# garrelt/C2-Ray3Dm

Hardware: AMD Instinct MI355X
Metric: cells-traced/sec (grid^3 x sources / wallclock) on 256^3 (higher is better)
Workload: dtype f64

## Files before the change

c2-ray3dm_amd/csrc/kernels_common.hpp:

```cpp
#pragma once
#include <hip/hip_runtime.h>
#include <stdint.h>

namespace c2r {

#ifndef C2R_BLOCK
#define C2R_BLOCK 256
#endif
constexpr int kFusedQmaxK = 10;
constexpr int kBlock = C2R_BLOCK;

typedef double v2f64 __attribute__((ext_vector_type(2)));
constexpr int kLogTab = 64;

struct ShellStep { double d2axis[3]; double path_scale, lls_scale; };
struct ChemStep { double dt, brech0, acolh0, recpow, clumping, sqrtt, expt, zp, dzdt; };
struct StepBlock {
    double dr[3], dr2[3], vol, coldensh_LLS, inv_dr0;
    int exact_udiv_dr0, n_shell;
    ChemStep chem;
};

struct KParams {
    int n[3];
// ... 5 lines not shown
    double inv_dlogtau;
    int exact_udiv;
    int numtau;
    int R, P;
    size_t PP;
    const double *nhi, *nhi_T;
    double *phih;
    double *phih_T;
    int lls_type;
    double R_max2;
    const float *lls, *lls_T;
    double *gbox_h;
    double *gbox;
    const double *thick, *thin;
    const double *hthick, *hthin;
    double *heat, *heat_T;
    double tau_heat_limit;
    const v2f64 *logtab;
    const v2f64 *odtab;
    double od_per_e, od_per_ln;
    const int    *srcpos;
    const int    *srcw;
    const double *normflux;
    const double *xthick, *xthin;
    const double *xhthick, *xhthin;
    const double *normflux_x;
    double *planes;
};

struct FaceRect {
    int a_lo, wa, b_lo, wb;
    unsigned magic;
    int ntiles;
    int pp, npr;
};

struct ShellArgs {
    int q;
    int has_boundary;
    int buf_prev, buf_cur;
    int tiles_max;
    int boxR[3], boxL[3];
    double alam;
    double dp2, inv_dp2;
    double inv_q;
    FaceRect face[6];
    const int *active;
    const int *n_active;
    double *loss_partial;
    double *dbg_cdout;
};

__device__ __forceinline__ int pmod(int a, int n) { int r = a % n; return r < 0 ? r + n : r; }

#define C2R_AS4 __attribute__((address_space(4)))
__device__ __forceinline__ const C2R_AS4 StepBlock &step_of(const KParams &p) { return *(const C2R_AS4 StepBlock *)p.step; }
__device__ __forceinline__ const C2R_AS4 ShellStep &shell_step(const KParams &p, int q) { return ((const C2R_AS4 ShellStep *)p.shell_step)[q]; }

__device__ __forceinline__ double rcp_nr(double d)
{
    double r = __builtin_amdgcn_rcp(d);
    double e = __builtin_fma(-d, r, 1.0);
    r = __builtin_fma(r, e, r);
    e = __builtin_fma(-d, r, 1.0);
    return __builtin_fma(r, e, r);
}
__device__ __forceinline__ double fdiv(double n, double d)
{
    const double r = rcp_nr(d);
    const double q = n * r;
    const double rem = __builtin_fma(-d, q, n);
    return __builtin_fma(rem, r, q);
}
__device__ __forceinline__ double frcp(double d)
{
    const double r = rcp_nr(d);
    const double rem = __builtin_fma(-d, r, 1.0);
    return __builtin_fma(rem, r, r);
}
__device__ __forceinline__ double fsqrt(double x)
{
#ifdef C2R_SQRT_GENERIC
    return sqrt(x);
#else
    const double y = __builtin_amdgcn_rsq(x);
    double g = x * y;
    double h = y * 0.5;
    const double r = __builtin_fma(-h, g, 0.5);
    g = __builtin_fma(g, r, g);
    h = __builtin_fma(h, r, h);
    double d = __builtin_fma(-g, g, x);
    g = __builtin_fma(d, h, g);
    d = __builtin_fma(-g, g, x);
    return __builtin_fma(d, h, g);
#endif
}
__device__ __forceinline__ double udiv(double n, double d, double rd, int exact)
{
    if (!exact) return n / d;
    const double q = n * rd;
    const double r = __builtin_fma(-q, d, n);
    return __builtin_fma(r, rd, q);
}

__device__ __forceinline__ double log10_pos(double x)
{
#ifdef C2R_LOG10_OCML
    return log10(x);
#else
    double m = __builtin_amdgcn_frexp_mant(x);
    int e = __builtin_amdgcn_frexp_exp(x);
    const bool lo = m < 0.70710678118654752440;
    m = lo ? m + m : m;
    e = lo ? e - 1 : e;
    const double dk = (double)e;
    const double f = m - 1.0;
    const double s = f * rcp_nr(2.0 + f);
    const double z = s * s, w = z * z;
    const double t1 = w * __builtin_fma(w, __builtin_fma(w, 1.531383769920937332e-01, 2.222219843214978396e-01),
                                        3.999999999940941908e-01);
    const double t2 = z * __builtin_fma(w, __builtin_fma(w, __builtin_fma(w, 1.479819860511658591e-01,
                                        1.818357216161805012e-01), 2.857142874366239149e-01),
                                        6.666666666666735130e-01);
    const double R = t2 + t1;
    const double hfsq = 0.5 * f * f;
    const double lm = f - (hfsq - s * (hfsq + R));
    const double hi = __builtin_fma(lm, 4.34294481903251816668e-01, dk * 3.01029995663611771306e-01);
    return __builtin_fma(dk, 3.69423907715893078616e-13, hi);
#endif
}

__device__ __forceinline__ double log10_tab(double x, const v2f64 *__restrict__ tab)
{
    const double m = __builtin_amdgcn_frexp_mant(x);
    const int e = __builtin_amdgcn_frexp_exp(x);
    const unsigned i = ((unsigned)__double2hiint(m) >> 14) & 63u;
    const v2f64 rt = tab[i];
    const double z = __builtin_fma(m, rt.x, -1.0);
    double P = __builtin_fma(z, 1.0 / 7.0, -1.0 / 6.0);
    P = __builtin_fma(z, P, 0.2);
    P = __builtin_fma(z, P, -0.25);
    P = __builtin_fma(z, P, 1.0 / 3.0);
    P = __builtin_fma(z, P, -0.5);
    const double l1p = __builtin_fma(z * z, P, z);
    return __builtin_fma((double)e, 3.01029995663981198017e-01, __builtin_fma(l1p, 4.34294481903251816668e-01, rt.y));
}
__device__ __forceinline__ const v2f64 *wave_log_table(const v2f64 *__restrict__ g, v2f64 *lds )
{
    const unsigned tid = threadIdx.x, lane = tid & 63u;
    v2f64 *mine = lds + (tid & ~63u);
    mine[lane] = g[lane];
    return mine;
}

struct TauPos { int ip, ip1; double res; };
__device__ __forceinline__ TauPos tau_pos(double tau, const KParams &p, const v2f64 *__restrict__ ltab)
{
#ifdef C2R_LOG10_NOTAB
    const double lt = log10_pos(fmax(1.0e-20, tau));
#else
    const double lt = log10_tab(fmax(1.0e-20, tau), ltab);
#endif
    const double od = fmin(p.numtau_d, fmax(0.0, 1.0 + udiv(lt - p.minlogtau, p.dlogtau, p.inv_dlogtau, p.exact_udiv)));
    TauPos t;
    t.ip = (int)od;
    t.res = od - (double)t.ip;
    t.ip1 = min(p.numtau, t.ip + 1);
    return t;
}
__device__ __forceinline__ double read_table(const double *__restrict__ tab, const TauPos &t)
{
    typedef double d2u __attribute__((ext_vector_type(2), aligned(8)));
    const d2u v = *reinterpret_cast<const d2u *>(tab + t.ip);
    return v.x + (v.y - v.x) * t.res;
}

template <int EXT = 0>
__device__ __forceinline__ double photoion(const KParams &p, const v2f64 *__restrict__ ltab, double cd_in, double cd_out,
                                           double vol_ph, double nflux, double &p_out, double *heat = nullptr, double nflux_x = 0.0)
{
    const double tau_in = cd_in * p.sigma, tau_out = cd_out * p.sigma;
    const TauPos pin = tau_pos(tau_in, p, ltab);
    const double p_in = nflux * read_table(p.thick, pin);
    double p_cell;
    TauPos pout = pin;
    const bool thick_cell = fabs(tau_out - tau_in) > p.tau_limit;
    if (thick_cell) {
        pout = tau_pos(tau_out, p, ltab);
        p_out = nflux * read_table(p.thick, pout);
        p_cell = p_in - p_out;
    } else {
        p_cell = nflux * (tau_out - tau_in) * read_table(p.thin, pin);
        p_out = p_in - p_cell;
    }
    if (EXT & 1) {
        const double h_in = nflux * read_table(p.hthick, pin);
        if (fabs(tau_out - tau_in) > p.tau_heat_limit) {
            if (!thick_cell) pout = tau_pos(tau_out, p, ltab);
            *heat = fdiv(h_in - nflux * read_table(p.hthick, pout), vol_ph);
        } else {
            const double tau_cell = (cd_out - cd_in) * p.sigma;
            *heat = fdiv(nflux * tau_cell * read_table(p.hthin, pin), vol_ph);
        }
    }
    double rate = fdiv(p_cell, vol_ph);
    if ((EXT & 2) && nflux_x > 0.0) {
        const double x_in = nflux_x * read_table(p.xthick, pin);
        double x_cell, x_out;
        if (thick_cell) {
            x_out = nflux_x * read_table(p.xthick, pout);
            x_cell = x_in - x_out;
        } else {
            x_cell = nflux_x * (tau_out - tau_in) * read_table(p.xthin, pin);
            x_out = x_in - x_cell;
        }
        p_out = p_out + x_out;
        rate = rate + fdiv(x_cell, vol_ph);
        if (EXT & 1) {
            const double hx_in = nflux_x * read_table(p.xhthick, pin);
            if (fabs(tau_out - tau_in) > p.tau_heat_limit) *heat = *heat + fdiv(hx_in - nflux_x * read_table(p.xhthick, pout), vol_ph);
            else *heat = *heat + fdiv(nflux_x * ((cd_out - cd_in) * p.sigma) * read_table(p.xhthin, pin), vol_ph);
        }
    }
    return rate;
}

__device__ __forceinline__ double block_sum_256(double v, double *sm )
{
    for (int off = 32; off > 0; off >>= 1) v += __shfl_down(v, off, 64);
    const int tid = threadIdx.y * blockDim.x + threadIdx.x;
    const int wave = tid >> 6, lane = tid & 63;
    if (lane == 0) sm[wave] = v;
    __syncthreads();
    double r = 0.0;
    if (tid == 0) { const int nw = (blockDim.x * blockDim.y) >> 6; for (int w = 0; w < nw; ++w) r += sm[w]; }
    return r;
}

__device__ __forceinline__ double rcp1(double d)
{
    const double r = __builtin_amdgcn_rcp(d);
    return __builtin_fma(__builtin_fma(-d, r, 1.0), r, r);
}
__device__ __forceinline__ double tau_od(double tau, const KParams &p, const v2f64 *__restrict__ tab)
{
    const double x = fmax(1.0e-20, tau);
    const double m = __builtin_amdgcn_frexp_mant(x);
    const int e = __builtin_amdgcn_frexp_exp(x);
    const unsigned i = ((unsigned)__double2hiint(m) >> 14) & 63u;
    const v2f64 rt = tab[i];
    const double z = __builtin_fma(m, rt.x, -1.0);
    double P = __builtin_fma(z, 1.0 / 7.0, -1.0 / 6.0);
    P = __builtin_fma(z, P, 0.2);
    P = __builtin_fma(z, P, -0.25);
    P = __builtin_fma(z, P, 1.0 / 3.0);
    P = __builtin_fma(z, P, -0.5);
    const double l1p = __builtin_fma(z * z, P, z);
    const double od = __builtin_fma((double)e, p.od_per_e, __builtin_fma(l1p, p.od_per_ln, rt.y));
    return fmin(p.numtau_d, od);
}
__device__ __forceinline__ double table_at(const double *__restrict__ tab, double od)
{
    typedef double d2u __attribute__((ext_vector_type(2), aligned(8)));
    const d2u v = *reinterpret_cast<const d2u *>(tab + (int)od);
    return __builtin_fma(v.y - v.x, __builtin_amdgcn_fract(od), v.x);
}

template <int EXT>
__device__ __forceinline__ double rates_fast(const KParams &p, const v2f64 *__restrict__ ltab, const double *__restrict__ thick,
                                             const double cd_in, const double cd_out, const double nflux, const double nflux_x,
                                             const double volnhi, const double vol_ph, double &p_out, double &heat)
{
    const double tau_in = cd_in * p.sigma, tau_out = cd_out * p.sigma;
    const double od_in = tau_od(tau_in, p, ltab);
    const double t_in = table_at(thick, od_in);
    double dT, t_out, od_out = od_in;
    const bool thick_cell = fabs(tau_out - tau_in) > p.tau_limit;
    if (thick_cell) {
        od_out = tau_od(tau_out, p, ltab);
        t_out = table_at(thick, od_out);
        dT = t_in - t_out;
    } else {
        dT = (tau_out - tau_in) * table_at(p.thin, od_in);
        t_out = t_in - dT;
    }
    p_out = nflux * t_out;
    if (EXT & 1) {
        const double h_in = table_at(p.hthick, od_in);
        double dH;
        if (fabs(tau_out - tau_in) > p.tau_heat_limit) {
            if (!thick_cell) od_out = tau_od(tau_out, p, ltab);
            dH = h_in - table_at(p.hthick, od_out);
        } else dH = ((cd_out - cd_in) * p.sigma) * table_at(p.hthin, od_in);
        heat = (nflux * dH) * rcp1(vol_ph);
    }
    const double r = rcp1(volnhi);
    double gamma = (nflux * dT) * r;
    if ((EXT & 2) && nflux_x > 0.0) {
        const double x_in = table_at(p.xthick, od_in);
        double dX, x_out;
        if (thick_cell) { x_out = table_at(p.xthick, od_out); dX = x_in - x_out; }
        else { dX = (tau_out - tau_in) * table_at(p.xthin, od_in); x_out = x_in - dX; }
        p_out = p_out + nflux_x * x_out;
        gamma = gamma + (nflux_x * dX) * r;
        if (EXT & 1) {
            double dHx;
            if (fabs(tau_out - tau_in) > p.tau_heat_limit) dHx = table_at(p.xhthick, od_in) - table_at(p.xhthick, od_out);
            else dHx = ((cd_out - cd_in) * p.sigma) * table_at(p.xhthin, od_in);
            heat = heat + (nflux_x * dHx) * rcp1(vol_ph);
        }
    }
    return gamma;
}

typedef unsigned v2u32 __attribute__((ext_vector_type(2)));
constexpr unsigned kOOB = 0x80000000u;
__device__ __forceinline__ __amdgpu_buffer_rsrc_t make_rsrc(const void *base, unsigned bytes)
{
    return __builtin_amdgcn_make_buffer_rsrc(const_cast<void *>(base), 0, (int)bytes, 0x00020000);
}
template <int AUX = 0>
__device__ __forceinline__ double buf_load_f64(__amdgpu_buffer_rsrc_t r, unsigned byte_off)
{
    return __builtin_bit_cast(double, __builtin_amdgcn_raw_buffer_load_b64(r, (int)byte_off, 0, AUX));
}
__device__ __forceinline__ float buf_load_f32(__amdgpu_buffer_rsrc_t r, unsigned byte_off)
{
    return __builtin_bit_cast(float, __builtin_amdgcn_raw_buffer_load_b32(r, (int)byte_off, 0, 0));
}
#ifndef C2R_STORE_AUX
#define C2R_STORE_AUX 2
#endif
#ifndef C2R_NHI_AUX
#define C2R_NHI_AUX 2
#endif
#ifndef C2R_PLANE_AUX
#define C2R_PLANE_AUX 2
#endif
template <int AUX = 0>
__device__ __forceinline__ void buf_store_f64(__amdgpu_buffer_rsrc_t r, unsigned byte_off, double v)
{
    __builtin_amdgcn_raw_buffer_store_b64(__builtin_bit_cast(v2u32, v), r, (int)byte_off, 0, AUX);
}

__device__ __forceinline__ unsigned wrap_pos(int srcw, int n, int d)
{
    unsigned c = (unsigned)(srcw + n + d);
    c = min(c, c - (unsigned)n);
    return min(c, c - (unsigned)n);
}

}
```

c2-ray3dm_amd/csrc/kernels_sweep.hpp:

```cpp
#pragma once
#include "kernels_common.hpp"

namespace c2r {

template <int EXT>
__device__ __forceinline__ void source_cell(const KParams &p, const v2f64 *__restrict__ ltab, const int s, const bool on_surface,
                                            double *loss_acc, double *dbg_cdout)
{
    const int i = pmod(p.srcpos[3 * s + 0] - 1, p.n[0]);
    const int j = pmod(p.srcpos[3 * s + 1] - 1, p.n[1]);
    const int k = pmod(p.srcpos[3 * s + 2] - 1, p.n[2]);
    const size_t id = (size_t)i + (size_t)p.n[0] * ((size_t)j + (size_t)p.n[1] * (size_t)k);
    const double nhi = p.nhi[id];
    const double cd_in = 0.0;
    const double path = 0.5 * step_of(p).dr[0];
    const double vol_ph = step_of(p).dr[0] * step_of(p).dr[1] * step_of(p).dr[2];
    const double cd_out = cd_in + nhi * path;
    for (int f = 0; f < 6; ++f)
        p.planes[((size_t)s * 2 + 0) * 6 * p.PP + (size_t)f * p.PP + (size_t)p.R * p.P + p.R] = cd_out;
    if (dbg_cdout) dbg_cdout[id] = cd_out;
    const double nflux = p.normflux[s];
    double p_out = 0.0, gamma = 0.0;
    if (nflux > 0.0) {
        double heat = 0.0;
// ... 369 lines not shown
        cdi = (abs(a) == 1 && abs(b) == 1) ? p.sqrt3 * cdi : p.sqrt2 * cdi;
    c.pq = sqrt_pos((double)(q * q + a2 + b * b));
    const C2R_AS4 ShellStep &ss = shell_step(p, q);
    c.path = c.pq * ss.path_scale;
    if (LLS == 3) c.cd_in = cdi;
    else if (LLS == 2) c.cd_in = __builtin_fma(lls_cell * sa.inv_q, c.pq, cdi);
    else c.cd_in = __builtin_fma(ss.lls_scale, c.pq, cdi);
    c.np = nhi * c.path;
    c.cd_out = c.cd_in + c.np;
    return c;
}

template <int LLS, bool STREAM>
__device__ __forceinline__ double lookahead_cd_out(const KParams &p, const ShellArgs &sq, const int face, const int s,
                                                   const int a, const int b)
{
    const int q = sq.q, qm = q - 1;
    const bool inside = abs(a) <= q && abs(b) <= q;
    const int axis = 2 - (face >> 1);
    const int pd = (face & 1) ? -q : q;
    int fo = face, ao = a, bo = b;
    if (axis == 1) { if (abs(b) == q) { fo = b > 0 ? 0 : 1; ao = a; bo = pd; } }
    else if (axis == 0) {
        if (abs(b) == q) { fo = b > 0 ? 0 : 1; ao = pd; bo = a; }
        else if (abs(a) == q) { fo = a > 0 ? 2 : 3; ao = pd; bo = b; }
    }
    const int sga = ao < 0 ? -1 : 1, sgb = bo < 0 ? -1 : 1;
    const int am = ao - sga, bm = bo - sgb;
    const unsigned plane_bytes = (unsigned)p.PP * 8u;
    const __amdgpu_buffer_rsrc_t r_prev = make_rsrc(p.planes + ((size_t)s * 2 + sq.buf_prev) * 6 * p.PP, 6u * plane_bytes);
    const bool ina = abs(ao) <= qm, inam = abs(am) <= qm, inb = abs(bo) <= qm, inbm = abs(bm) <= qm;
    const unsigned base = (unsigned)fo * plane_bytes;
    constexpr int PA = STREAM ? C2R_PLANE_AUX : 0;
    const double v_mm = buf_load_f64<PA>(r_prev, (inam && inbm) ? base + plane_off8(p, am, bm) : kOOB);
    const double v_am = buf_load_f64<PA>(r_prev, (ina && inbm) ? base + plane_off8(p, ao, bm) : kOOB);
    const double v_mb = buf_load_f64<PA>(r_prev, (inam && inb) ? base + plane_off8(p, am, bo) : kOOB);
    const double v_ab = buf_load_f64<PA>(r_prev, (ina && inb) ? base + plane_off8(p, ao, bo) : kOOB);
    const Delta3 dl = mesh_delta(axis, pd, a, b);
    const unsigned c0 = wrap_pos(p.srcw[3 * s + 0], p.n[0], dl.d0), c1 = wrap_pos(p.srcw[3 * s + 1], p.n[1], dl.d1),
                   c2 = wrap_pos(p.srcw[3 * s + 2], p.n[2], dl.d2);
    const unsigned id = c0 + (unsigned)p.n[0] * (c1 + (unsigned)p.n[1] * c2);
    const unsigned ncell = (unsigned)p.n[0] * (unsigned)p.n[1] * (unsigned)p.n[2];
    const double nhi = buf_load_f64<STREAM ? C2R_NHI_AUX : 0>(make_rsrc(p.nhi, ncell * 8u), id * 8u);
    const double omu = (double)abs(ao) * sq.inv_q, ddu = 1.0 - omu;
    double Rlo, Tlo, Rhi, Thi;
    row_sum_fast(p, omu, ddu, v_mm, v_am, Rlo, Tlo);
    row_sum_fast(p, omu, ddu, v_mb, v_ab, Rhi, Thi);
    const double cd_out = cell_cd_fast<LLS>(p, sq, ao, ao * ao, bo, Rlo, Tlo, Rhi, Thi, nhi, LLS == 2 ? (double)p.lls[id] : 0.0).cd_out;
    return inside ? cd_out : 0.0;
}

#ifndef C2R_XCD_KEEP_DBG
#define C2R_XCD_KEEP_DBG 0
#endif
constexpr int kLdsR = kFusedQmaxK, kLdsP = 2 * kFusedQmaxK + 1, kLdsPP = kLdsP * kLdsP;
template <bool DET, int LLS, int STREAM, int NR, int EXT, int STORE = 1>
__device__ __forceinline__ double shell_rows_fast_core(const KParams &p, const ShellArgs &sa, const v2f64 *__restrict__ ltab,
                                                       const double *__restrict__ thick, const int face, const int s, const int a,
                                                       const int b0, const int sgb, const int nvalid,
                                                       const double (&vm)[NR + 1], const double (&va_)[NR + 1],
                                                       double *__restrict__ lds_cur = nullptr)
{
    const int q = sa.q;
    const int axis = 2 - (face >> 1);
    const int pd = (face & 1) ? -q : q;
    const bool xf = (axis == 0);
    const int ua = xf ? 1 : 0, va = (axis == 2) ? 1 : 2;
    const unsigned plane_bytes = (unsigned)p.PP * 8u;
    const unsigned p8 = (unsigned)p.P * 8u;
    const unsigned db8 = sgb < 0 ? 0u - p8 : p8;
    const unsigned o_first = plane_off8(p, a, b0);
    const unsigned na = (unsigned)p.n[ua], nmid = xf ? (unsigned)p.n[0] : (unsigned)p.n[1];
    const unsigned ca = wrap_pos(p.srcw[3 * s + ua], p.n[ua], a);
    const unsigned cp = wrap_pos(p.srcw[3 * s + axis], p.n[axis], pd);
    const unsigned stride_b = (axis == 2) ? na : na * nmid;
    const unsigned base_p = (axis == 2) ? na * nmid * cp : na * cp;
    const unsigned ncell = (unsigned)p.n[0] * (unsigned)p.n[1] * (unsigned)p.n[2];
    const __amdgpu_buffer_rsrc_t r_x = make_rsrc(xf ? p.nhi_T : p.nhi, ncell * 8u);
    unsigned id[NR];
    double nhi[NR];
#pragma unroll
    for (int k = 0; k < NR; ++k) {
        const unsigned cb = wrap_pos(p.srcw[3 * s + va], p.n[va], b0 + k * sgb);
        id[k] = ca + base_p + __umul24(stride_b, cb);
        nhi[k] = buf_load_f64<STREAM == 1 ? C2R_NHI_AUX : 0>(r_x, id[k] * 8u);
    }
    const double omu = (double)abs(a) * sa.inv_q, ddu = 1.0 - omu;
    const int a2 = a * a;
    const double du2 = step_of(p).dr2[ua] * (double)a2;
    double R[NR + 1], T[NR + 1];
#pragma unroll
    for (int r = 0; r <= NR; ++r) row_sum_fast(p, omu, ddu, vm[r], va_[r], R[r], T[r]);
    const double nflux = p.normflux[s];
    const double nflux_x = (EXT & 2) ? p.normflux_x[s] : 0.0;
    const __amdgpu_buffer_rsrc_t r_cur = make_rsrc(p.planes + ((size_t)s * 2 + sa.buf_cur) * 6 * p.PP, 6u * plane_bytes);
    constexpr int SA = (STREAM & 1) ? C2R_STORE_AUX : 0;
    const bool bnd_col = sa.has_boundary && (a == sa.boxR[ua] || a == -sa.boxL[ua] || pd == sa.boxR[axis] || pd == -sa.boxL[axis]);
    double loss = 0.0;
    unsigned o8 = o_first;
#pragma unroll
    for (int k = 0; k < NR; ++k) {
        const int b = b0 + k * sgb;
        if (k < nvalid) {
            const CellCd cc = cell_cd_fast<LLS>(p, sa, a, a2, b, R[k], T[k], R[k + 1], T[k + 1], nhi[k],
                                                LLS == 2 ? (double)(xf ? p.lls_T : p.lls)[id[k]] : 0.0);
            const double path = cc.path, cd_in = cc.cd_in, np = cc.np, cd_out = cc.cd_out;
            const double dist2 = __builtin_fma(step_of(p).dr2[va], (double)(b * b), du2 + shell_step(p, q).d2axis[axis]);
            const bool stop = (LLS == 3) && dist2 > p.R_max2;
            if (STORE == 1) {
            buf_store_f64<SA>(r_cur, (unsigned)face * plane_bytes + o8, cd_out);
            if (axis == 2) {
                if (abs(a) == q)
                    buf_store_f64<SA>(r_cur, (a > 0 ? 4u : 5u) * plane_bytes + (unsigned)((pd + p.R) * p.P + (b + p.R)) * 8u, cd_out);
                if (abs(b) == q)
                    buf_store_f64<SA>(r_cur, (b > 0 ? 2u : 3u) * plane_bytes + (unsigned)((pd + p.R) * p.P + (a + p.R)) * 8u, cd_out);
            } else if (axis == 1) {
                if (abs(a) == q)
                    buf_store_f64<SA>(r_cur, (a > 0 ? 4u : 5u) * plane_bytes + (unsigned)((b + p.R) * p.P + (pd + p.R)) * 8u, cd_out);
            }
            }
            if (STORE == 2) {
                lds_cur[face * kLdsPP + (b + kLdsR) * kLdsP + (a + kLdsR)] = cd_out;
                if (axis == 2) {
                    if (abs(a) == q) lds_cur[(a > 0 ? 4 : 5) * kLdsPP + (pd + kLdsR) * kLdsP + (b + kLdsR)] = cd_out;
                    if (abs(b) == q) lds_cur[(b > 0 ? 2 : 3) * kLdsPP + (pd + kLdsR) * kLdsP + (a + kLdsR)] = cd_out;
                } else if (axis == 1) {
                    if (abs(a) == q) lds_cur[(a > 0 ? 4 : 5) * kLdsPP + (b + kLdsR) * kLdsP + (pd + kLdsR)] = cd_out;
                }
            }
            if ((C2R_XCD_KEEP_DBG || !(STREAM & 2)) && sa.dbg_cdout) {
                const Delta3 dl = mesh_delta(axis, pd, a, b);
                const unsigned c0 = wrap_pos(p.srcw[3 * s + 0], p.n[0], dl.d0), c1 = wrap_pos(p.srcw[3 * s + 1], p.n[1], dl.d1),
                               c2 = wrap_pos(p.srcw[3 * s + 2], p.n[2], dl.d2);
                sa.dbg_cdout[c0 + (unsigned)p.n[0] * (c1 + (unsigned)p.n[1] * c2)] = cd_out;
            }
            double gamma = 0.0, heat = 0.0;
            if (!stop && !(cd_in > p.max_coldensh) && nflux > 0.0) {
                const double area = p.fourpi * dist2;
                double p_out;
                gamma = rates_fast<EXT>(p, ltab, thick, cd_in, cd_out, nflux, nflux_x, area * np, area * path, p_out, heat);
                if (!DET && gamma != 0.0) atomicAdd(&(xf ? p.phih_T : p.phih)[id[k]], gamma);
                if ((EXT & 1) && !DET && heat != 0.0) atomicAdd(&(xf ? p.heat_T : p.heat)[id[k]], heat);
                if (sa.has_boundary && (bnd_col || b == sa.boxR[va] || b == -sa.boxL[va]))
                    loss = loss + fdiv(p_out * step_of(p).vol, area * path);
            }
            if (DET) p.gbox[((size_t)s * 2 + (xf ? 1 : 0)) * ncell + id[k]] = gamma;
            if (DET && (EXT & 1)) p.gbox_h[((size_t)s * 2 + (xf ? 1 : 0)) * ncell + id[k]] = heat;
        }
        o8 += db8;
    }
    return loss;
}

template <bool DET, int LLS, int STREAM, int NR, int EXT, int LOOK = 0, int STORE = 1>
__device__ __forceinline__ double shell_rows_fast(const KParams &p, const ShellArgs &sa, const v2f64 *__restrict__ ltab,
                                                  const double *__restrict__ thick,
                                                  const int face, const int s, const int a, const int b0, const int sgb,
                                                  const int nvalid, const ShellArgs &sq,
                                                  const double *__restrict__ lds_prev = nullptr, double *__restrict__ lds_cur = nullptr)
{
    const int q = sa.q, qm = q - 1;
    const int sga = a < 0 ? -1 : 1;
    const int am = a - sga;
    double vm[NR + 1], va_[NR + 1];
    if (LOOK == 2) {
        const bool ina = abs(a) <= qm, inam = abs(am) <= qm;
        const double *pl = lds_prev + face * kLdsPP + kLdsR * kLdsP + kLdsR;
#pragma unroll
        for (int r = 0; r <= NR; ++r) {
            const int row = b0 + (r - 1) * sgb;
            const bool inr = abs(row) <= qm;
            vm[r] = (inam && inr) ? pl[row * kLdsP + am] : 0.0;
            va_[r] = (ina && inr) ? pl[row * kLdsP + a] : 0.0;
        }
    } else if (LOOK) {
#pragma unroll
        for (int r = 0; r <= NR; ++r) {
            const int row = b0 + (r - 1) * sgb;
            vm[r] = lookahead_cd_out<LLS, (STREAM & 1) != 0>(p, sq, face, s, am, row);
            va_[r] = lookahead_cd_out<LLS, (STREAM & 1) != 0>(p, sq, face, s, a, row);
        }
    } else {
        const unsigned plane_bytes = (unsigned)p.PP * 8u;
        const __amdgpu_buffer_rsrc_t r_prev =
            make_rsrc(p.planes + ((size_t)s * 2 + sa.buf_prev) * 6 * p.PP + (size_t)face * p.PP, plane_bytes);
        const bool ina = abs(a) <= qm, inam = abs(am) <= qm;
        const unsigned p8 = (unsigned)p.P * 8u;
        const unsigned da8 = (unsigned)(sga * 8), db8 = sgb < 0 ? 0u - p8 : p8;
        unsigned o = plane_off8(p, a, b0) - db8;
#pragma unroll
        for (int r = 0; r <= NR; ++r) {
            const bool inr = abs(b0 + (r - 1) * sgb) <= qm;
            vm[r] = buf_load_f64<(STREAM & 1) ? C2R_PLANE_AUX : 0>(r_prev, (inam && inr) ? o - da8 : kOOB);
            va_[r] = buf_load_f64<(STREAM & 1) ? C2R_PLANE_AUX : 0>(r_prev, (ina && inr) ? o : kOOB);
            o += db8;
        }
    }
    return shell_rows_fast_core<DET, LLS, STREAM, NR, EXT, STORE>(p, sa, ltab, thick, face, s, a, b0, sgb, nvalid, vm, va_, lds_cur);
}

#ifndef C2R_FAST_ATTR
#define C2R_FAST_ATTR __launch_bounds__(kBlock)
#endif
template <bool DET, int LLS, int STREAM, int EXT, int LOOK = 0, int STORE = 1, int NR = kRows>
__device__ __forceinline__ void sweep_tile_fast(const KParams &p, const ShellArgs &sa, const FaceRect &fr, const v2f64 *ltab,
                                                const double *thick, double *sm, const int face, const int tile, const int sl,
                                                const ShellArgs &sq, const int src = -1)
{
    double loss = 0.0;
    const unsigned t = (unsigned)tile * kBlock + threadIdx.x;
    const unsigned bi = fr.magic ? __umulhi(t, fr.magic) : t;
    if (tile < fr.ntiles && bi < (unsigned)fr.npr) {
        const int a = fr.a_lo + (int)(t - __umul24(bi, (unsigned)fr.wa));
        const bool pos = bi < (unsigned)fr.pp;
        const int k0 = NR * (pos ? (int)bi : (int)bi - fr.pp);
        const int sgb = pos ? 1 : -1;
        const int b0 = pos ? k0 : -1 - k0;
        const int left = pos ? (fr.b_lo + fr.wb - b0) : (b0 - fr.b_lo + 1);
        loss = shell_rows_fast<DET, LLS, STREAM, NR, EXT, LOOK, STORE>(p, sa, ltab, thick, face, src < 0 ? sa.active[sl] : src, a, b0, sgb,
                                                                        min(left, NR), sq);
    }
    if (sa.has_boundary) {
        const double tot = block_sum_256(loss, sm);
        if (threadIdx.x == 0)
            sa.loss_partial[((size_t)sl * 6 + face) * sa.tiles_max + tile] = tot;
    }
}

template <bool DET, int LLS, bool STREAM, int EXT>
__global__ C2R_FAST_ATTR void k_sweep_shell_fast(KParams p, ShellArgs sa)
{
    __shared__ double sm[16];
    __shared__ v2f64 s_log[kBlock];
    const int face = blockIdx.y;
    const int tile = blockIdx.x;
    const int nact = *sa.n_active;
    if ((int)blockIdx.z >= nact) return;
    const FaceRect fr = sa.face[face];
    if (tile >= fr.ntiles && !sa.has_boundary) return;
    const v2f64 *ltab = wave_log_table(p.odtab, s_log);
    sweep_tile_fast<DET, LLS, STREAM, EXT>(p, sa, fr, ltab, p.thick, sm, face, tile, (int)blockIdx.z, sa);
}

struct XcdArgs {
    const int *perm;
    int n, cap;
    const int *final_nbox;
};
template <bool DET, int LLS, bool STREAM, int EXT, bool FAST>
__global__ C2R_FAST_ATTR void k_sweep_shell_xcd(KParams p, ShellArgs sa, XcdArgs xa)
{
    __shared__ double sm[16];
    __shared__ v2f64 s_log[kBlock];
    const unsigned x = blockIdx.x & 7u;
    unsigned r = blockIdx.x >> 3;
    const unsigned start = (x * (unsigned)xa.n) >> 3, cnt = (((x + 1u) * (unsigned)xa.n) >> 3) - start;
    int face = -1; unsigned item = 0, tile = 0;
#pragma unroll
    for (int f = 0; f < 6; ++f) {
        const unsigned nt = (unsigned)sa.face[f].ntiles, nb = cnt * nt;
        if (face < 0) {
            if (r < nb) { face = f; item = r / nt; tile = r - item * nt; }
            else r -= nb;
        }
    }
    if (face < 0) return;
    const int s = xa.perm[(2 - (face >> 1)) * xa.cap + (int)(start + item)];
    if (xa.final_nbox[s] != 0) return;
    const FaceRect fr = sa.face[face];
    const v2f64 *ltab = wave_log_table(p.odtab, s_log);
    if (FAST) sweep_tile_fast<DET, LLS, STREAM ? 3 : 2, EXT>(p, sa, fr, ltab, p.thick, sm, face, (int)tile, 0, sa, s);
    else sweep_tile<DET, LLS, STREAM ? 3 : 2, EXT>(p, sa, fr, ltab, sm, face, (int)tile, 0, sa, s);
}

template <bool DET, int LLS, bool STREAM, int EXT>
__global__ __launch_bounds__(kBlock) __attribute__((amdgpu_waves_per_eu(1, 4)))
void k_sweep_pair_fast(KParams p, ShellArgs sa, ShellArgs sb)
{
    __shared__ double sm[16];
    __shared__ v2f64 s_log[kBlock];
    const bool second = blockIdx.y >= 6;
    const int face = second ? (int)blockIdx.y - 6 : (int)blockIdx.y;
    const int tile = blockIdx.x;
    const int nact = *sa.n_active;
    if ((int)blockIdx.z >= nact) return;
    const v2f64 *ltab = (C2R_PAIR_LDS_TABLE) ? wave_log_table(p.odtab, s_log) : p.odtab;
    if (second) {
        const FaceRect fr = sb.face[face];
        if (tile >= fr.ntiles) return;
        sweep_tile_fast<DET, LLS, STREAM, EXT, 1, true, kPairRows>(p, sb, fr, ltab, p.thick, sm, face, tile, (int)blockIdx.z, sa);
    } else {
        const FaceRect fr = sa.face[face];
        if (tile >= fr.ntiles) return;
        sweep_tile_fast<DET, LLS, STREAM, EXT, 0, false>(p, sa, fr, ltab, p.thick, sm, face, tile, (int)blockIdx.z, sa);
    }
}

constexpr int kMaxFused = 5;
struct BoxArgs {
    int source_cell;
    int nshell;
    int ncell[kMaxFused];
    int face_off[kMaxFused][8];
    ShellArgs sh[kMaxFused];
    const int *active;
    const int *n_active;
    double *loss_acc;
};

template <bool DET, int LLS, bool FAST, int EXT>
__global__ __launch_bounds__(1024) void k_sweep_box_fused(KParams p, BoxArgs ba)
{
    __shared__ double sm[16];
    __shared__ v2f64 s_log[1024];
#ifdef C2R_FUSED_NO_LDS
    constexpr bool kLdsPlanes = false;
#else
    constexpr bool kLdsPlanes = FAST;
#endif
    __shared__ double s_planes[kLdsPlanes ? 2 * 6 * kLdsPP : 1];
    const int sl = blockIdx.x;
    if (sl >= *ba.n_active) return;
    const int s = ba.active[sl];
    const v2f64 *ltab = wave_log_table(p.odtab, s_log);
    if (ba.source_cell) {
        if (threadIdx.x == 0) {
            const ShellArgs &s0 = ba.sh[0];
            source_cell<EXT>(p, p.logtab, s, s0.boxR[0] == 0 || s0.boxR[1] == 0 || s0.boxR[2] == 0 || s0.boxL[0] == 0 ||
                              s0.boxL[1] == 0 || s0.boxL[2] == 0, ba.loss_acc, s0.dbg_cdout);
        }
        __syncthreads();
    }
    for (int k = 0; k < ba.nshell; ++k) {
        const ShellArgs &sa = ba.sh[k];
        double loss = 0.0;
        for (int t = threadIdx.x; t < ba.ncell[k]; t += blockDim.x) {
            int f = 0;
#pragma unroll
            for (int g = 1; g < 6; ++g) f += (t >= ba.face_off[k][g]) ? 1 : 0;
            const FaceRect fr = sa.face[f];
            const unsigned lt = (unsigned)(t - ba.face_off[k][f]);
            const unsigned bi = fr.magic ? __umulhi(lt, fr.magic) : lt;
            const int a = fr.a_lo + (int)(lt - __umul24(bi, (unsigned)fr.wa));
            const int b = fr.b_lo + (int)bi;
            if (FAST && !kLdsPlanes) loss = loss + shell_rows_fast<DET, LLS, false, 1, EXT>(p, sa, ltab, p.thick, f, s, a, b, b < 0 ? -1 : 1, 1, sa);
            else if (FAST) {
                const double *lp = s_planes + ((k - 1) & 1) * 6 * kLdsPP;
                double *lc = s_planes + (k & 1) * 6 * kLdsPP;
                const int sg = b < 0 ? -1 : 1;
                if (k == 0) {
                    if (k + 1 < ba.nshell) loss = loss + shell_rows_fast<DET, LLS, false, 1, EXT, 0, 2>(p, sa, ltab, p.thick, f, s, a, b, sg, 1, sa, nullptr, lc);
                    else loss = loss + shell_rows_fast<DET, LLS, false, 1, EXT, 0, 1>(p, sa, ltab, p.thick, f, s, a, b, sg, 1, sa);
                } else {
                    if (k + 1 < ba.nshell) loss = loss + shell_rows_fast<DET, LLS, false, 1, EXT, 2, 2>(p, sa, ltab, p.thick, f, s, a, b, sg, 1, sa, lp, lc);
                    else loss = loss + shell_rows_fast<DET, LLS, false, 1, EXT, 2, 1>(p, sa, ltab, p.thick, f, s, a, b, sg, 1, sa, lp, nullptr);
                }
            } else loss = loss + shell_cell<DET, LLS, 0, EXT>(p, sa, ltab, f, s, a, b);
        }
        if (sa.has_boundary) {
            const double tot = block_sum_256(loss, sm);
            if (threadIdx.x == 0) ba.loss_acc[s] += tot;
        }
        __syncthreads();
    }
}

__global__ __launch_bounds__(256) void k_gamma_reduce(KParams p, int nsrc, const int *final_nbox, int subbox,
                                                      double *phih, double *heat ,
                                                      const int *gate = nullptr )
{
    if (gate && *gate != 0) return;
    const int c0 = blockIdx.x * 8 + (threadIdx.x & 7), c1 = blockIdx.y * 32 + (threadIdx.x >> 3), c2 = blockIdx.z;
    const bool live = c0 < p.n[0] && c1 < p.n[1];
    const unsigned ncell = (unsigned)p.n[0] * (unsigned)p.n[1] * (unsigned)p.n[2];
    const unsigned id = (unsigned)c0 + (unsigned)p.n[0] * ((unsigned)c1 + (unsigned)p.n[1] * (unsigned)c2);
    const unsigned id_t = (unsigned)c1 + (unsigned)p.n[1] * ((unsigned)c0 + (unsigned)p.n[0] * (unsigned)c2);
    double acc = live ? phih[id] : 0.0;
    double acc_h = (live && heat) ? heat[id] : 0.0;
    for (int s = 0; s < nsrc; ++s) {
        const int nb = final_nbox[s];
        if (nb <= 0) continue;
        const int ext = subbox * nb;
        int d2 = c2 - p.srcw[3 * s + 2];
        d2 -= (d2 > p.hr[2]) ? p.n[2] : 0;  d2 += (d2 < -p.hl[2]) ? p.n[2] : 0;
        if (d2 < -min(ext, p.hl[2]) || d2 > min(ext, p.hr[2])) continue;
        int d0 = c0 - p.srcw[3 * s + 0], d1 = c1 - p.srcw[3 * s + 1];
        d0 -= (d0 > p.hr[0]) ? p.n[0] : 0;  d0 += (d0 < -p.hl[0]) ? p.n[0] : 0;
        d1 -= (d1 > p.hr[1]) ? p.n[1] : 0;  d1 += (d1 < -p.hl[1]) ? p.n[1] : 0;
        if (live && d0 >= -min(ext, p.hl[0]) && d0 <= min(ext, p.hr[0]) && d1 >= -min(ext, p.hl[1]) && d1 <= min(ext, p.hr[1])) {
            const bool xf = abs(d0) > max(abs(d1), abs(d2));
            const double *g = p.gbox + ((size_t)s * 2 + (xf ? 1 : 0)) * ncell;
            acc = acc + g[xf ? id_t : id];
            if (heat) acc_h = acc_h + (p.gbox_h + ((size_t)s * 2 + (xf ? 1 : 0)) * ncell)[xf ? id_t : id];
        }
    }
    if (live) phih[id] = acc;
    if (live && heat) heat[id] = acc_h;
}

struct ZeroGrids { double *g[4]; };
struct WordCopy { const unsigned *src; unsigned *dst; unsigned n; };
__global__ __launch_bounds__(256) void k_prepare_nhi(int n0, int n1, int n2, double eps, const float *__restrict__ ndens,
                                                     const double *__restrict__ xh_av, double *__restrict__ nhi,
                                                     double *__restrict__ nhi_T, ZeroGrids zero, WordCopy copy,
                                                     const double *__restrict__ xh_av0 = nullptr )
{
    __shared__ double tile[32][33];
    const int k = blockIdx.z;
    if (copy.n && blockIdx.x == 0 && blockIdx.y == 0 && k == 0)
        for (unsigned w = threadIdx.x; w < copy.n; w += 256) copy.dst[w] = copy.src[w];
    const int i0 = blockIdx.x * 32, j0 = blockIdx.y * 32;
    const int tx = threadIdx.x & 31, ty = threadIdx.x >> 5;
    for (int r = ty; r < 32; r += 8) {
        const int i = i0 + tx, j = j0 + r;
        if (i < n0 && j < n1) {
            const size_t id = (size_t)i + (size_t)n0 * ((size_t)j + (size_t)n1 * k);
            const double xav1 = fmax(xh_av[id], eps);
            const double xav0 = xh_av0 ? fmax(xh_av0[id], eps)
                                       : fmax(1.0 - xav1, eps);
            const double v = xav0 * (double)ndens[id];
            nhi[id] = v;
            tile[r][tx] = v;
// ... 233 lines not shown
```

profiles/isa_count.py:

```python
#!/usr/bin/env python3
import os
import re
import subprocess
import sys
from collections import Counter

ROOT = os.path.dirname(os.path.dirname(os.path.abspath(__file__)))
SRC = os.path.join(ROOT, "c2-ray3dm_amd", "csrc", "sweep.hip")
FLAGS = "--offload-arch=gfx950 -O3 -std=c++17 -fPIC -ffp-contract=off -munsafe-fp-atomics".split()


def main():
    pats = sys.argv[1:] or ["k_sweep_shell_fastILb0ELi1ELb1", "k_sweep_shellILb0ELi1ELb1"]
    extra = os.environ.get("C2R_EXTRA_FLAGS", "").split()
    out = "/tmp/c2r_isa.s"
    subprocess.check_call(["/opt/rocm/bin/hipcc"] + FLAGS + extra + ["-S", "--cuda-device-only", "-o", out, SRC],
                          stderr=subprocess.DEVNULL)
    lines = open(out).read().split("\n")
    starts = [(i, l.split(":")[0]) for i, l in enumerate(lines) if re.match(r"^_Z\w+:", l)]
    for n, (i, name) in enumerate(starts):
        if not any(p in name for p in pats):
            continue
        c = Counter()
        for l in lines[i + 1:]:
            t = l.strip()
            if t.startswith(".Lfunc_end"):
                break
            if not t or t[0] in ";." or t.endswith(":"):
                continue
            c[t.split()[0]] += 1
        grp = lambda pred: sum(v for k, v in c.items() if pred(k))
        valu = grp(lambda k: k.startswith("v_"))
        f64 = grp(lambda k: k.startswith("v_") and "f64" in k)
        trans = grp(lambda k: k in ("v_rcp_f64_e32", "v_rsq_f64_e32", "v_rcp_f64_e64", "v_rsq_f64_e64"))
        print("%s\n  VALU %d (f64 %d, of them rcp/rsq %d)  SALU %d  SMEM %d  buffer/global %d  LDS %d" %
              (name, valu, f64, trans, grp(lambda k: k.startswith("s_") and not k.startswith("s_load") and not k.startswith("s_buffer")),
               grp(lambda k: k.startswith("s_load") or k.startswith("s_buffer")),
               grp(lambda k: k.startswith(("buffer_", "global_", "flat_"))), grp(lambda k: k.startswith("ds_"))))
        top = sorted(((v, k) for k, v in c.items() if k.startswith("v_")), reverse=True)[:24]
        print("  " + "  ".join("%s:%d" % (k, v) for v, k in top))


if __name__ == "__main__":
    main()
```

Baseline: 122.3 billion.

## Restructure fast shell rows into issue/front/consume/commit phases for memory-level parallelism

Adds an ordered variant of the fast shell-row path for EXT==0 that issues all plane and nhi loads up front, then runs per-row front (log/tau and table-pair gathers), consume (lerp and rates) and commit (stores and atomics) phases. All table gathers are in flight before they are used. The per-wave LDS log-table fill is split into an issue and a finish step, so the global load overlaps with the row loads. This is meant to hide memory latency, at the cost of more live registers and possible occupancy loss. It also adds an optional waves-per-EU attribute and an ISA memory-order dump in the profiling script.

```diff
diff --git a/c2-ray3dm_amd/csrc/kernels_common.hpp b/c2-ray3dm_amd/csrc/kernels_common.hpp
--- a/c2-ray3dm_amd/csrc/kernels_common.hpp
+++ b/c2-ray3dm_amd/csrc/kernels_common.hpp
@@ -181,6 +181,20 @@
     mine[lane] = g[lane];
     return mine;
 }
+struct LogFill { v2f64 v; v2f64 *mine; };
+__device__ __forceinline__ LogFill wave_log_table_issue(const v2f64 *__restrict__ g, v2f64 *lds )
+{
+    const unsigned tid = threadIdx.x;
+    LogFill f;
+    f.v = g[tid & 63u];
+    f.mine = lds + (tid & ~63u);
+    return f;
+}
+__device__ __forceinline__ const v2f64 *wave_log_table_finish(const LogFill &f)
+{
+    f.mine[threadIdx.x & 63u] = f.v;
+    return f.mine;
+}
 
 struct TauPos { int ip, ip1; double res; };
 __device__ __forceinline__ TauPos tau_pos(double tau, const KParams &p, const v2f64 *__restrict__ ltab)
@@ -288,12 +302,10 @@
     const double od = __builtin_fma((double)e, p.od_per_e, __builtin_fma(l1p, p.od_per_ln, rt.y));
     return fmin(p.numtau_d, od);
 }
-__device__ __forceinline__ double table_at(const double *__restrict__ tab, double od)
-{
-    typedef double d2u __attribute__((ext_vector_type(2), aligned(8)));
-    const d2u v = *reinterpret_cast<const d2u *>(tab + (int)od);
-    return __builtin_fma(v.y - v.x, __builtin_amdgcn_fract(od), v.x);
-}
+typedef double d2u __attribute__((ext_vector_type(2), aligned(8)));
+__device__ __forceinline__ d2u table_pair(const double *tab, double od) { return *reinterpret_cast<const d2u *>(tab + (int)od); }
+__device__ __forceinline__ double pair_lerp(const d2u v, double frac) { return __builtin_fma(v.y - v.x, frac, v.x); }
+__device__ __forceinline__ double table_at(const double *__restrict__ tab, double od) { return pair_lerp(table_pair(tab, od), __builtin_amdgcn_fract(od)); }
 
 template <int EXT>
 __device__ __forceinline__ double rates_fast(const KParams &p, const v2f64 *__restrict__ ltab, const double *__restrict__ thick,
diff --git a/c2-ray3dm_amd/csrc/kernels_sweep.hpp b/c2-ray3dm_amd/csrc/kernels_sweep.hpp
--- a/c2-ray3dm_amd/csrc/kernels_sweep.hpp
+++ b/c2-ray3dm_amd/csrc/kernels_sweep.hpp
@@ -545,6 +545,235 @@
     return loss;
 }
 
+#ifndef C2R_MEMORDER
+#define C2R_MEMORDER 2
+#endif
+template <int EXT> constexpr bool kOrdered = C2R_MEMORDER != 0 && EXT == 0;
+template <int STREAM, int NR>
+__device__ __forceinline__ void rows_nhi_issue(const KParams &p, const ShellArgs &sa, const int face, const int s, const int a,
+                                               const int b0, const int sgb, unsigned (&id)[NR], double (&nhi)[NR])
+{
+    const int axis = 2 - (face >> 1);
+    const int pd = (face & 1) ? -sa.q : sa.q;
+    const bool xf = (axis == 0);
+    const int ua = xf ? 1 : 0, va = (axis == 2) ? 1 : 2;
+    const unsigned na = (unsigned)p.n[ua], nmid = xf ? (unsigned)p.n[0] : (unsigned)p.n[1];
+    const unsigned ca = wrap_pos(p.srcw[3 * s + ua], p.n[ua], a);
+    const unsigned cp = wrap_pos(p.srcw[3 * s + axis], p.n[axis], pd);
+    const unsigned stride_b = (axis == 2) ? na : na * nmid;
+    const unsigned base_p = (axis == 2) ? na * nmid * cp : na * cp;
+    const unsigned ncell = (unsigned)p.n[0] * (unsigned)p.n[1] * (unsigned)p.n[2];
+    const __amdgpu_buffer_rsrc_t r_x = make_rsrc(xf ? p.nhi_T : p.nhi, ncell * 8u);
+#pragma unroll
+    for (int k = 0; k < NR; ++k) {
+        const unsigned cb = wrap_pos(p.srcw[3 * s + va], p.n[va], b0 + k * sgb);
+        id[k] = ca + base_p + __umul24(stride_b, cb);
+        nhi[k] = buf_load_f64<STREAM == 1 ? C2R_NHI_AUX : 0>(r_x, id[k] * 8u);
+    }
+}
+template <bool DET, int LLS, int STREAM, int NR, int EXT, int STORE, int ORD>
+__device__ __forceinline__ double shell_rows_fast_ordered(const KParams &p, const ShellArgs &sa, const v2f64 *__restrict__ ltab,
+                                                          const double *__restrict__ thick, const int face, const int s, const int a,
+                                                          const int b0, const int sgb, const int nvalid,
+                                                          const double (&vm)[NR + 1], const double (&va_)[NR + 1],
+                                                          const unsigned (&id)[NR], const double (&nhi)[NR],
+                                                          double *__restrict__ lds_cur = nullptr)
+{
+    const int q = sa.q;
+    const int axis = 2 - (face >> 1);
+    const int pd = (face & 1) ? -q : q;
+    const bool xf = (axis == 0);
+    const int ua = xf ? 1 : 0, va = (axis == 2) ? 1 : 2;
+    const unsigned plane_bytes = (unsigned)p.PP * 8u;
+    const unsigned p8 = (unsigned)p.P * 8u;
+    const unsigned db8 = sgb < 0 ? 0u - p8 : p8;
+    const unsigned o_first = plane_off8(p, a, b0);
+    const unsigned ncell = (unsigned)p.n[0] * (unsigned)p.n[1] * (unsigned)p.n[2];
+    const double omu = (double)abs(a) * sa.inv_q, ddu = 1.0 - omu;
+    const int a2 = a * a;
+    const double du2 = step_of(p).dr2[ua] * (double)a2;
+    double R[NR + 1], T[NR + 1];
+#pragma unroll
+    for (int r = 0; r <= NR; ++r) row_sum_fast(p, omu, ddu, vm[r], va_[r], R[r], T[r]);
+    const double nflux = p.normflux[s];
+    const double nflux_x = (EXT & 2) ? p.normflux_x[s] : 0.0;
+    const __amdgpu_buffer_rsrc_t r_cur = make_rsrc(p.planes + ((size_t)s * 2 + sa.buf_cur) * 6 * p.PP, 6u * plane_bytes);
+    constexpr int SA = (STREAM & 1) ? C2R_STORE_AUX : 0;
+    constexpr bool BND = !(STREAM & 2);
+    const bool bnd_col = BND && sa.has_boundary && (a == sa.boxR[ua] || a == -sa.boxL[ua] || pd == sa.boxR[axis] || pd == -sa.boxL[axis]);
+    double loss = 0.0;
+
+    double cd_out[NR], od_in[NR], dtau[NR], f1[NR], u2[NR], fh[NR], dtauh[NR], volnhi[NR], vol_ph[NR], gamma[NR], heat[NR];
+    bool live[NR], thk[NR], hthk[NR];
+    d2u P1[NR], P2[NR], H1[NR], H2[NR], X1[NR], X2[NR], XH1[NR], XH2[NR];
+
+    auto front = [&](const int k) __attribute__((always_inline)) {
+        const int b = b0 + k * sgb;
+        const CellCd cc = cell_cd_fast<LLS>(p, sa, a, a2, b, R[k], T[k], R[k + 1], T[k + 1], nhi[k],
+                                            LLS == 2 ? (double)(xf ? p.lls_T : p.lls)[id[k]] : 0.0);
+        cd_out[k] = cc.cd_out;
+        const double dist2 = __builtin_fma(step_of(p).dr2[va], (double)(b * b), du2 + shell_step(p, q).d2axis[axis]);
+        const bool stop = (LLS == 3) && dist2 > p.R_max2;
+        live[k] = k < nvalid && !stop && !(cc.cd_in > p.max_coldensh) && nflux > 0.0;
+        const double area = p.fourpi * dist2;
+        volnhi[k] = area * cc.np;
+        vol_ph[k] = area * cc.path;
+        const double tau_in = cc.cd_in * p.sigma, tau_out = cc.cd_out * p.sigma;
+        od_in[k] = live[k] ? tau_od(tau_in, p, ltab) : 1.0;
+        dtau[k] = tau_out - tau_in;
+        if (EXT & 1) dtauh[k] = (cc.cd_out - cc.cd_in) * p.sigma;
+        thk[k] = fabs(dtau[k]) > p.tau_limit;
+        hthk[k] = (EXT & 1) && fabs(dtau[k]) > p.tau_heat_limit;
+        const bool need = live[k] && (thk[k] || hthk[k]);
+        double od_out = od_in[k];
+        if (__any(need)) {
+            const double o = tau_od(tau_out, p, ltab);
+            od_out = need ? o : od_out;
+        }
+        const double pos2 = thk[k] ? od_out : od_in[k], posh = hthk[k] ? od_out : od_in[k];
+        P1[k] = table_pair(thick, od_in[k]);
+        P2[k] = table_pair(thk[k] ? thick : p.thin, pos2);
+        if (EXT & 1) {
+            H1[k] = table_pair(p.hthick, od_in[k]);
+            H2[k] = table_pair(hthk[k] ? p.hthick : p.hthin, posh);
+        }
+        if (EXT & 2) {
+            X1[k] = table_pair(p.xthick, od_in[k]);
+            X2[k] = table_pair(thk[k] ? p.xthick : p.xthin, pos2);
+        }
+        if (EXT == 3) {
+            XH1[k] = table_pair(p.xhthick, od_in[k]);
+            XH2[k] = table_pair(hthk[k] ? p.xhthick : p.xhthin, posh);
+        }
+        f1[k] = __builtin_amdgcn_fract(od_in[k]);
+        u2[k] = thk[k] ? __builtin_amdgcn_fract(od_out) : dtau[k];
+        if (EXT & 1) fh[k] = __builtin_amdgcn_fract(posh);
+    };
+    auto consume = [&](const int k) __attribute__((always_inline)) {
+        const int b = b0 + k * sgb;
+        const double f2 = thk[k] ? u2[k] : f1[k], dt = u2[k];
+        const double t_in = pair_lerp(P1[k], f1[k]);
+        const double v2 = pair_lerp(P2[k], f2);
+        const double dT = thk[k] ? t_in - v2 : dt * v2;
+        const double t_out = thk[k] ? v2 : t_in - dT;
+        double p_out = nflux * t_out;
+        double h = 0.0;
+        if (EXT & 1) {
+            const double h_in = pair_lerp(H1[k], f1[k]);
+            const double hv = pair_lerp(H2[k], fh[k]);
+            const double dH = hthk[k] ? h_in - hv : dtauh[k] * hv;
+            h = (nflux * dH) * rcp1(vol_ph[k]);
+        }
+        const double r = rcp1(volnhi[k]);
+        double g = (nflux * dT) * r;
+        if ((EXT & 2) && nflux_x > 0.0) {
+            const double x_in = pair_lerp(X1[k], f1[k]);
+            const double xv = pair_lerp(X2[k], f2);
+            const double dX = thk[k] ? x_in - xv : dt * xv;
+            const double x_out = thk[k] ? xv : x_in - dX;
+            p_out = p_out + nflux_x * x_out;
+            g = g + (nflux_x * dX) * r;
+            if (EXT & 1) {
+                const double xh_in = pair_lerp(XH1[k], f1[k]);
+                const double xhv = pair_lerp(XH2[k], fh[k]);
+                const double dHx = hthk[k] ? xh_in - xhv : dtauh[k] * xhv;
+                h = h + (nflux_x * dHx) * rcp1(vol_ph[k]);
+            }
+        }
+        gamma[k] = live[k] ? g : 0.0;
+        heat[k] = live[k] ? h : 0.0;
+        if (BND && sa.has_boundary && live[k] && (bnd_col || b == sa.boxR[va] || b == -sa.boxL[va]))
+            loss = loss + fdiv(p_out * step_of(p).vol, vol_ph[k]);
+    };
+    auto commit = [&](const int k) __attribute__((always_inline)) {
+        const int b = b0 + k * sgb;
+        const unsigned o8 = o_first + (unsigned)k * db8;
+        if (k < nvalid) {
+            if (STORE == 1) {
+                buf_store_f64<SA>(r_cur, (unsigned)face * plane_bytes + o8, cd_out[k]);
+                if (axis == 2) {
+                    if (abs(a) == q)
+                        buf_store_f64<SA>(r_cur, (a > 0 ? 4u : 5u) * plane_bytes + (unsigned)((pd + p.R) * p.P + (b + p.R)) * 8u, cd_out[k]);
+                    if (abs(b) == q)
+                        buf_store_f64<SA>(r_cur, (b > 0 ? 2u : 3u) * plane_bytes + (unsigned)((pd + p.R) * p.P + (a + p.R)) * 8u, cd_out[k]);
+                } else if (axis == 1) {
+                    if (abs(a) == q)
+                        buf_store_f64<SA>(r_cur, (a > 0 ? 4u : 5u) * plane_bytes + (unsigned)((b + p.R) * p.P + (pd + p.R)) * 8u, cd_out[k]);
+                }
+            }
+            if (STORE == 2) {
+                lds_cur[face * kLdsPP + (b + kLdsR) * kLdsP + (a + kLdsR)] = cd_out[k];
+                if (axis == 2) {
+                    if (abs(a) == q) lds_cur[(a > 0 ? 4 : 5) * kLdsPP + (pd + kLdsR) * kLdsP + (b + kLdsR)] = cd_out[k];
+                    if (abs(b) == q) lds_cur[(b > 0 ? 2 : 3) * kLdsPP + (pd + kLdsR) * kLdsP + (a + kLdsR)] = cd_out[k];
+                } else if (axis == 1) {
+                    if (abs(a) == q) lds_cur[(a > 0 ? 4 : 5) * kLdsPP + (b + kLdsR) * kLdsP + (pd + kLdsR)] = cd_out[k];
+                }
+            }
+            if ((C2R_XCD_KEEP_DBG || !(STREAM & 2)) && sa.dbg_cdout) {
+                const Delta3 dl = mesh_delta(axis, pd, a, b);
+                const unsigned c0 = wrap_pos(p.srcw[3 * s + 0], p.n[0], dl.d0), c1 = wrap_pos(p.srcw[3 * s + 1], p.n[1], dl.d1),
+                               c2 = wrap_pos(p.srcw[3 * s + 2], p.n[2], dl.d2);
+                sa.dbg_cdout[c0 + (unsigned)p.n[0] * (c1 + (unsigned)p.n[1] * c2)] = cd_out[k];
+            }
+            if (DET) p.gbox[((size_t)s * 2 + (xf ? 1 : 0)) * ncell + id[k]] = gamma[k];
+            if (DET && (EXT & 1)) p.gbox_h[((size_t)s * 2 + (xf ? 1 : 0)) * ncell + id[k]] = heat[k];
+        }
+        if (!DET && gamma[k] != 0.0) atomicAdd(&(xf ? p.phih_T : p.phih)[id[k]], gamma[k]);
+        if ((EXT & 1) && !DET && heat[k] != 0.0) atomicAdd(&(xf ? p.heat_T : p.heat)[id[k]], heat[k]);
+    };
+
+    if (ORD == 2) {
+#pragma unroll
+        for (int k = 0; k < NR; ++k) front(k);
+#pragma unroll
+        for (int k = 0; k < NR; ++k) consume(k);
+#pragma unroll
+        for (int k = 0; k < NR; ++k) commit(k);
+    } else if (ORD == 3) {
+        front(0);
+#pragma unroll
+        for (int k = 0; k < NR; ++k) {
+            if (k + 1 < NR) front(k + 1);
+            consume(k);
+        }
+#pragma unroll
+        for (int k = 0; k < NR; ++k) commit(k);
+    } else {
+        front(0);
+#pragma unroll
+        for (int k = 0; k < NR; ++k) {
+            consume(k);
+            if (k + 1 < NR) front(k + 1);
+            commit(k);
+        }
+    }
+    return loss;
+}
+
+template <int STREAM, int NR>
+__device__ __forceinline__ void rows_planes_issue(const KParams &p, const ShellArgs &sa, const int face, const int s, const int a,
+                                                  const int b0, const int sgb, double (&vm)[NR + 1], double (&va_)[NR + 1])
+{
+    const int qm = sa.q - 1;
+    const int sga = a < 0 ? -1 : 1;
+    const int am = a - sga;
+    const unsigned plane_bytes = (unsigned)p.PP * 8u;
+    const __amdgpu_buffer_rsrc_t r_prev =
+        make_rsrc(p.planes + ((size_t)s * 2 + sa.buf_prev) * 6 * p.PP + (size_t)face * p.PP, plane_bytes);
+    const bool ina = abs(a) <= qm, inam = abs(am) <= qm;
+    const unsigned p8 = (unsigned)p.P * 8u;
+    const unsigned da8 = (unsigned)(sga * 8), db8 = sgb < 0 ? 0u - p8 : p8;
+    unsigned o = plane_off8(p, a, b0) - db8;
+#pragma unroll
+    for (int r = 0; r <= NR; ++r) {
+        const bool inr = abs(b0 + (r - 1) * sgb) <= qm;
+        vm[r] = buf_load_f64<(STREAM & 1) ? C2R_PLANE_AUX : 0>(r_prev, (inam && inr) ? o - da8 : kOOB);
+        va_[r] = buf_load_f64<(STREAM & 1) ? C2R_PLANE_AUX : 0>(r_prev, (ina && inr) ? o : kOOB);
+        o += db8;
+    }
+}
+
 template <bool DET, int LLS, int STREAM, int NR, int EXT, int LOOK = 0, int STORE = 1>
 __device__ __forceinline__ double shell_rows_fast(const KParams &p, const ShellArgs &sa, const v2f64 *__restrict__ ltab,
                                                   const double *__restrict__ thick,
@@ -573,27 +802,22 @@
             vm[r] = lookahead_cd_out<LLS, (STREAM & 1) != 0>(p, sq, face, s, am, row);
             va_[r] = lookahead_cd_out<LLS, (STREAM & 1) != 0>(p, sq, face, s, a, row);
         }
-    } else {
-        const unsigned plane_bytes = (unsigned)p.PP * 8u;
-        const __amdgpu_buffer_rsrc_t r_prev =
-            make_rsrc(p.planes + ((size_t)s * 2 + sa.buf_prev) * 6 * p.PP + (size_t)face * p.PP, plane_bytes);
-        const bool ina = abs(a) <= qm, inam = abs(am) <= qm;
-        const unsigned p8 = (unsigned)p.P * 8u;
-        const unsigned da8 = (unsigned)(sga * 8), db8 = sgb < 0 ? 0u - p8 : p8;
-        unsigned o = plane_off8(p, a, b0) - db8;
-#pragma unroll
-        for (int r = 0; r <= NR; ++r) {
-            const bool inr = abs(b0 + (r - 1) * sgb) <= qm;
-            vm[r] = buf_load_f64<(STREAM & 1) ? C2R_PLANE_AUX : 0>(r_prev, (inam && inr) ? o - da8 : kOOB);
-            va_[r] = buf_load_f64<(STREAM & 1) ? C2R_PLANE_AUX : 0>(r_prev, (ina && inr) ? o : kOOB);
-            o += db8;
-        }
-    }
-    return shell_rows_fast_core<DET, LLS, STREAM, NR, EXT, STORE>(p, sa, ltab, thick, face, s, a, b0, sgb, nvalid, vm, va_, lds_cur);
+    } else rows_planes_issue<STREAM, NR>(p, sa, face, s, a, b0, sgb, vm, va_);
+    if constexpr (kOrdered<EXT>) {
+        unsigned id[NR];
+        double nhi[NR];
+        rows_nhi_issue<STREAM, NR>(p, sa, face, s, a, b0, sgb, id, nhi);
+        return shell_rows_fast_ordered<DET, LLS, STREAM, NR, EXT, STORE, C2R_MEMORDER>(p, sa, ltab, thick, face, s, a, b0, sgb, nvalid, vm, va_, id, nhi, lds_cur);
+    } else
+        return shell_rows_fast_core<DET, LLS, STREAM, NR, EXT, STORE>(p, sa, ltab, thick, face, s, a, b0, sgb, nvalid, vm, va_, lds_cur);
 }
 
 #ifndef C2R_FAST_ATTR
+#ifdef C2R_FAST_WAVES
+#define C2R_FAST_ATTR __launch_bounds__(kBlock) __attribute__((amdgpu_waves_per_eu(C2R_FAST_WAVES, 8)))
+#else
 #define C2R_FAST_ATTR __launch_bounds__(kBlock)
+#endif
 #endif
 template <bool DET, int LLS, int STREAM, int EXT, int LOOK = 0, int STORE = 1, int NR = kRows>
 __device__ __forceinline__ void sweep_tile_fast(const KParams &p, const ShellArgs &sa, const FaceRect &fr, const v2f64 *ltab,
@@ -620,6 +844,39 @@
     }
 }
 
+template <bool DET, int LLS, int STREAM, int EXT>
+__device__ __forceinline__ void sweep_tile_far(const KParams &p, const ShellArgs &sa, const FaceRect &fr, const LogFill &lf,
+                                               double *sm, const int face, const int tile, const int sl, const int src = -1)
+{
+    constexpr int NR = kRows;
+    double loss = 0.0;
+    const unsigned t = (unsigned)tile * kBlock + threadIdx.x;
+    const unsigned bi = fr.magic ? __umulhi(t, fr.magic) : t;
+    const bool act = tile < fr.ntiles && bi < (unsigned)fr.npr;
+    const int a = fr.a_lo + (int)(t - __umul24(bi, (unsigned)fr.wa));
+    const bool pos = bi < (unsigned)fr.pp;
+    const int k0 = NR * (pos ? (int)bi : (int)bi - fr.pp);
+    const int sgb = pos ? 1 : -1;
+    const int b0 = pos ? k0 : -1 - k0;
+    const int left = pos ? (fr.b_lo + fr.wb - b0) : (b0 - fr.b_lo + 1);
+    const int s = src < 0 ? sa.active[sl] : src;
+    double vm[NR + 1], va_[NR + 1], nhi[NR];
+    unsigned id[NR];
+    if (act) {
+        rows_planes_issue<STREAM, NR>(p, sa, face, s, a, b0, sgb, vm, va_);
+        rows_nhi_issue<STREAM, NR>(p, sa, face, s, a, b0, sgb, id, nhi);
+    }
+    const v2f64 *ltab = wave_log_table_finish(lf);
+    if (act)
+        loss = shell_rows_fast_ordered<DET, LLS, STREAM, NR, EXT, 1, C2R_MEMORDER>(p, sa, ltab, p.thick, face, s, a, b0, sgb, min(left, NR),
+                                                                                    vm, va_, id, nhi);
+    if (sa.has_boundary) {
+        const double tot = block_sum_256(loss, sm);
+        if (threadIdx.x == 0)
+            sa.loss_partial[((size_t)sl * 6 + face) * sa.tiles_max + tile] = tot;
+    }
+}
+
 template <bool DET, int LLS, bool STREAM, int EXT>
 __global__ C2R_FAST_ATTR void k_sweep_shell_fast(KParams p, ShellArgs sa)
 {
@@ -631,8 +888,11 @@
     if ((int)blockIdx.z >= nact) return;
     const FaceRect fr = sa.face[face];
     if (tile >= fr.ntiles && !sa.has_boundary) return;
-    const v2f64 *ltab = wave_log_table(p.odtab, s_log);
-    sweep_tile_fast<DET, LLS, STREAM, EXT>(p, sa, fr, ltab, p.thick, sm, face, tile, (int)blockIdx.z, sa);
+    if constexpr (kOrdered<EXT>) sweep_tile_far<DET, LLS, STREAM, EXT>(p, sa, fr, wave_log_table_issue(p.odtab, s_log), sm, face, tile, (int)blockIdx.z);
+    else {
+        const v2f64 *ltab = wave_log_table(p.odtab, s_log);
+        sweep_tile_fast<DET, LLS, STREAM, EXT>(p, sa, fr, ltab, p.thick, sm, face, tile, (int)blockIdx.z, sa);
+    }
 }
 
 struct XcdArgs {
@@ -661,6 +921,7 @@
     const int s = xa.perm[(2 - (face >> 1)) * xa.cap + (int)(start + item)];
     if (xa.final_nbox[s] != 0) return;
     const FaceRect fr = sa.face[face];
+    if constexpr (FAST && kOrdered<EXT>) { sweep_tile_far<DET, LLS, STREAM ? 3 : 2, EXT>(p, sa, fr, wave_log_table_issue(p.odtab, s_log), sm, face, (int)tile, 0, s); return; }
     const v2f64 *ltab = wave_log_table(p.odtab, s_log);
     if (FAST) sweep_tile_fast<DET, LLS, STREAM ? 3 : 2, EXT>(p, sa, fr, ltab, p.thick, sm, face, (int)tile, 0, sa, s);
     else sweep_tile<DET, LLS, STREAM ? 3 : 2, EXT>(p, sa, fr, ltab, sm, face, (int)tile, 0, sa, s);
diff --git a/profiles/isa_count.py b/profiles/isa_count.py
--- a/profiles/isa_count.py
+++ b/profiles/isa_count.py
@@ -10,16 +10,46 @@
 FLAGS = "--offload-arch=gfx950 -O3 -std=c++17 -fPIC -ffp-contract=off -munsafe-fp-atomics".split()
 
 
+def memory_order(lines, i):
+    nv = 0
+    for l in lines[i + 1:]:
+        t = l.strip()
+        if t.startswith(".Lfunc_end"):
+            break
+        if not t or t[0] in ";.":
+            if t.startswith(".LBB") and t.split()[0].endswith(":"):
+                print("    %s" % t.split()[0])
+            continue
+        op = t.split()[0]
+        if op.startswith("v_"):
+            nv += 1
+        show = op.startswith(("buffer_", "global_", "flat_", "ds_write")) or (op == "s_waitcnt" and "vmcnt" in t)
+        if show:
+            print("    [+%3d valu] %s" % (nv, re.sub(r"\s+", " ", t.split(";")[0])[:100]))
+            nv = 0
+    end = next(j for j in range(i, len(lines)) if lines[j].strip().startswith(".Lfunc_end"))
+    for l in lines[end:end + 80]:
+        if re.match(r"^; (NumVgprs|NumAgprs|ScratchSize|Occupancy):", l):
+            print("    " + l[2:].strip())
+
+
 def main():
+    order = "--order" in sys.argv[1:]
+    if order:
+        sys.argv.remove("--order")
     pats = sys.argv[1:] or ["k_sweep_shell_fastILb0ELi1ELb1", "k_sweep_shellILb0ELi1ELb1"]
     extra = os.environ.get("C2R_EXTRA_FLAGS", "").split()
-    out = "/tmp/c2r_isa.s"
+    out = os.environ.get("C2R_ISA_OUT", "/tmp/c2r_isa.s")
     subprocess.check_call(["/opt/rocm/bin/hipcc"] + FLAGS + extra + ["-S", "--cuda-device-only", "-o", out, SRC],
                           stderr=subprocess.DEVNULL)
     lines = open(out).read().split("\n")
     starts = [(i, l.split(":")[0]) for i, l in enumerate(lines) if re.match(r"^_Z\w+:", l)]
     for n, (i, name) in enumerate(starts):
         if not any(p in name for p in pats):
+            continue
+        if order:
+            print(name)
+            memory_order(lines, i)
             continue
         c = Counter()
         for l in lines[i + 1:]:
```

After: 122.6 billion, median of 6. No clear change (+0.2%).
